# sunwj/SunVolumeRender

Measured on AMD Instinct MI355X. Metric: Msamples/sec (paths x spp) at 1024^2 on 512^3 volume, higher is better.
Workload: dtype f32; 1 GPU; c3: 512^3 u16 CT-like volume, 1024x1024 image, 3 area lights, env map on, trace depth 1, 256 spp per step; math=bit-exact contract, parallelism=single GPU

## Files before the change

sunvolumerender_amd/csrc/svr_api.hip:

```cpp
#include "../../include/svr_abi.h"
#include "svr_kernels.hpp"
#include "svr_denoise.hpp"
#include "svr_noise.hpp"
#include "svr_project.hpp"
#include "svr_slice.hpp"
#include "svr_hits.hpp"
#include "svr_device.hpp"

#include <hip/hip_runtime.h>
#include <algorithm>
#include <cmath>
#include <cstdarg>
#include <cstdio>
#include <cstdlib>
#include <cstring>
#include <dlfcn.h>
#include <mutex>
#include <string>
#include <unordered_map>
#include <vector>

static_assert(sizeof(svr_vec3) == 12, "glm::vec3 layout");
static_assert(sizeof(svr_bbox) == 36, "cudaBBox layout");
static_assert(sizeof(svr_volume) == 112 && offsetof(svr_volume, tex) == 40 && offsetof(svr_volume, densityScale) == 48 &&
// ... 91 lines not shown
        uint32_t first = 0, count = 0, depth = 0;
        int set = -1;
    } ahead[2];
    uint64_t content_version = 0;
    int opt_frame_ahead = 1;
#ifndef SVR_GROUP
#define SVR_GROUP 32
#endif
    static constexpr int NSETS = 4, GROUP = SVR_GROUP;
    static constexpr int AHEAD_MAX = 64;
    static constexpr uint64_t CHAIN_MIN_PATHS = 12u << 20;
    struct SlotSet {
        float* lbuf = nullptr;
        hipStream_t stream = nullptr;
        hipEvent_t traced = nullptr, resolved = nullptr;
        bool used = false;
        float4* planes[svr::WF_QUEUE_PLANES] = {};
        uint32_t* wf_counts = nullptr;
    } sets[NSETS];
    size_t queue_capacity = 0;
    size_t slot_floats = 0;
    uint32_t slots_per_set = 0;
    int next_set = 0;
    int opt_pipeline = 1, opt_refill = 16, opt_empty_skip = 1, opt_ray_skip = 1, opt_debug_stop = 0, opt_frames_log2 = -1, opt_unit = 0, opt_rc_lanes = 3, opt_bound_cull = 1, opt_park_end = 32, opt_fold = 1, opt_queue = 1, opt_fast_math = 0, opt_fine_mask = 0, opt_row_order = 0, opt_group_frames = 64, opt_local_majorant = 0, opt_light_cull = 1, opt_lm_tune = 0, opt_lm_sub = 1, opt_park_cheap = 16, opt_pinhole_fast = 1, opt_pool = 1, opt_trips = 1, opt_nan_guard = 0, opt_macro_shift_min = 0, opt_split = 0, opt_env_nee = 0, opt_fast_bound = 1;
    uint32_t* d_mask = nullptr;
    uint32_t* d_fine_mask = nullptr;
    size_t fine_mask_words = 0;
    uint8_t* d_bnd8 = nullptr;
    uint8_t* d_sub8 = nullptr;
    bool sub8_valid = false;
    bool bnd8_valid = false;
    uint8_t* d_mask_tmp = nullptr;
    uint32_t* d_pick = nullptr;
    bool mask_valid = false;
    uint64_t mask_vol = 0, mask_tf = 0, mask_tf_version = 0;
    uint32_t mask_ds_bits = 0, mask_sigma_bits = 0;
    bool mask_cull_useful = false, mask_has_empty = true;
    uint32_t mask_words = 0;
    int opt_denoise_preview = 0;
    svr_denoise_params dn = DN_DEFAULT;
    float4* d_guides = nullptr;
    size_t guides_px = 0;
    bool guides_valid = false;
    svr::DevScene guides_key{};
    uint64_t guides_vol = 0, guides_tf = 0, guides_tf_version = 0;
    float guides_h = 0.f;
    int guides_skip = -1;
// ... 519 lines not shown
        if (!st.wf_counts) HIP_TRY(hipMalloc((void**)&st.wf_counts, 64 * sizeof(uint32_t)));
    }
    if (need >= ((size_t)1 << 31)) return fail(-3, "frame too large for the wavefront queues");
    for (auto& st : g.sets)
        for (auto& p : st.planes) HIP_TRY(hipMalloc((void**)&p, need * sizeof(float4)));
    g.queue_capacity = need;
    return 0;
}

struct TileList {
    const uint32_t* list = nullptr;
    uint32_t count = 0;
    const uint8_t* active = nullptr;
};

struct LaunchPlan {
    svr::DevScene s;
    svr::LaunchCfg cfg;
    void* img = nullptr;
    const svr_render_params* rp = nullptr;
    const TileList* tiles = nullptr;
    bool fold_batch = false;
    bool use_queue = false;
    bool local_majorant = false;
    bool frame_ahead = false;
};

constexpr uint32_t FOLD_MIN = 8;

int plan_launch(LaunchPlan& p, void* img, const svr_render_params* rp, uint32_t nframes, const TileList* adaptive)
{
    svr::DevScene& s = p.s;
    svr::LaunchCfg& cfg = p.cfg;
    p.img = img;
    p.rp = rp;
    p.tiles = adaptive != nullptr && adaptive->list != nullptr ? adaptive : nullptr;
    if (build_scene(g.vol, g.tf, g.cam, s)) return g.err_code;
    if (add_lights_env(s)) return g.err_code;
    if ((size_t)3 * s.imageW * s.imageH >= ((size_t)1 << 32)) return fail(-3, "image too large");
    if (rp->frameNo == 0 && partial_frame(s.imageW, s.imageH))
        HIP_TRY(hipMemsetAsync(rp->hdrBuffer, 0, sizeof(float) * 3 * (size_t)s.imageW * s.imageH, g.stream));
    cfg.kernel = g.opt_kernel == svr::KERNEL_AUTO ? svr::KERNEL_TILE : g.opt_kernel;
    if (g.opt_env_nee && cfg.kernel == svr::KERNEL_TILE && s.env != nullptr && s.env_cdf != nullptr && s.env_on_escape && rp->traceDepth >= 2 && !g.opt_debug_stop)
        cfg.kernel = svr::KERNEL_ENV_NEE;
    if ((cfg.kernel == svr::KERNEL_TILE || cfg.kernel == svr::KERNEL_WAVEFRONT || cfg.kernel == svr::KERNEL_ENV_NEE) && ensure_mask(s, g.vol, g.tf)) return g.err_code;
    if (cfg.kernel == svr::KERNEL_WAVEFRONT) {
// ... 6 lines not shown
    cfg.frames_log2 = g.opt_frames_log2;
    cfg.unit_override = g.opt_unit;
    cfg.lm_straight = g.opt_local_majorant == 2;
    cfg.pool_primary = false;
    p.fold_batch = cfg.kernel == svr::KERNEL_TILE && g.opt_fold && !g.opt_debug_stop && cfg.frames_log2 < 0;
    p.use_queue = p.fold_batch && g.opt_queue == 2;
    if (p.fold_batch && g.opt_queue == 1 && g.opt_empty_skip) {
        svr::DevWork wq;
        fill_work(wq, s.imageW, s.imageH);
        const uint64_t waves = (uint64_t)(cfg.num_cus * cfg.blocks_per_cu) / 4u * svr::TILE_WAVES;
        p.use_queue = rp->traceDepth >= 2 || s.bound_cull || (uint64_t)wq.n_items >= svr::QUEUE_AUTO_TASKS_PER_WAVE * waves;
    }
    p.local_majorant = g.opt_local_majorant && cfg.kernel == svr::KERNEL_TILE && s.empty_mask != nullptr && s.ray_skip && !g.opt_debug_stop;
    if (p.local_majorant && !g.opt_lm_tune && rp->traceDepth > 1) s.lm_tune = 2u | (32u << 8) | (48u << 16) | (s.lm_tune & 0xff000000u);
    if (p.local_majorant) p.use_queue = false;
    cfg.pool_primary = p.use_queue && (g.opt_pool == 2 || (g.opt_pool == 1 && s.bound_cull && !s.has_empty));
    if (p.use_queue || (p.local_majorant && p.fold_batch)) {
        bool available = true;
        if (ensure_record_queues((uint32_t)(cfg.num_cus * cfg.blocks_per_cu) * 4u / 16u, g.opt_queue == 1 && !p.local_majorant, available)) return g.err_code;
        p.use_queue = p.use_queue && available;
    }
    p.frame_ahead = nframes == 1 && g.opt_frame_ahead && g.opt_pipeline && !g.opt_count && !g.opt_debug_stop && cfg.kernel == svr::KERNEL_TILE &&
                    adaptive == nullptr;
    const uint32_t tail_frames = nframes % (uint32_t)(p.fold_batch ? g.opt_group_frames : Context::GROUP);
    if ((!p.fold_batch || p.frame_ahead || (tail_frames != 0 && tail_frames < FOLD_MIN)) &&
        ensure_slots(s.imageW, s.imageH, nframes < (uint32_t)Context::GROUP ? nframes : (uint32_t)Context::GROUP)) return g.err_code;
    return 0;
}

svr::DevWork launch_work(const LaunchPlan& p, uint32_t first, uint32_t n, bool want_img)
{
    svr::DevWork w;
    fill_work(w, p.s.imageW, p.s.imageH);
    w.hdr = (float*)p.rp->hdrBuffer;
    w.img = want_img ? (uint8_t*)p.img : nullptr;
    w.traceDepth = p.rp->traceDepth;
    w.frame0 = first;
    w.nframes = n;
    if (p.tiles) {
        w.tile_list = p.tiles->list;
        w.tile_count = p.tiles->count;
        w.tile_active = p.tiles->active;
        w.row_order = 0;
    }
    return w;
}

// ... 104 lines not shown
        svr::DevWork w = launch_work(p, n, 1, want_img);
        w.slot_stride = (uint32_t)g.slot_floats;
        w.lbuf = set.lbuf + (size_t)(n - a.first) * g.slot_floats;
        HIP_TRY(hipStreamWaitEvent(g.stream, set.traced, 0));
        HIP_TRY(svr::launch_resolve(s, w, g.stream));
        HIP_TRY(hipEventRecord(set.resolved, g.stream));
        const uint32_t next_first = a.first + a.count;
        const uint32_t next_count = 2u * a.count < batch_max ? 2u * a.count : batch_max;
        if (next_count > 1u && !in_stock(g.ahead[0], next_first) && !in_stock(g.ahead[1], next_first))
            return trace_group(p, next_set(), next_first, next_count, 0, false, ahead_queue && next_count >= 16u);
        return 0;
    }
    uint32_t batch = 1;
    while (batch < batch_max && 2u * batch <= n + 1u) batch *= 2u;
    if (batch_max > 1 && ensure_slots(s.imageW, s.imageH, batch_max)) return g.err_code;
    if (trace_group(p, next_set(), n, batch, 1, want_img, ahead_queue && batch >= 16u)) return g.err_code;
    if (batch_max > 1) {
        const uint32_t next_count = 2u * batch < batch_max ? 2u * batch : batch_max;
        return trace_group(p, next_set(), n + batch, next_count, 0, false, ahead_queue && next_count >= 16u);
    }
    return 0;
}

int render_frames_traced(void* img, const svr_render_params* rp, uint32_t nframes, bool tonemap, const TileList* adaptive)
{
    if (ensure_init()) return g.err_code;
    if (!rp) return fail(-4, "render_pathtracer: renderParams is null");
    if (!g.have_vol || !g.have_tf || !g.have_cam)
        return fail(-4, "render_pathtracer before setup_volume/setup_transferfunction/setup_camera");
    if (!rp->hdrBuffer) return fail(-4, "render_pathtracer: renderParams.hdrBuffer is null (call SetupHDRBuffer)");
    if (nframes == 0) return 0;
    LaunchPlan p;
    if (plan_launch(p, img, rp, nframes, adaptive)) return g.err_code;
    const bool want_img = tonemap && !g.opt_skip_tonemap;
    if (p.frame_ahead) return render_ahead(p, want_img);
    const uint32_t group = p.fold_batch ? (uint32_t)g.opt_group_frames : (uint32_t)Context::GROUP;
    for (uint32_t g0 = 0; g0 < nframes; g0 += group) {
        const uint32_t n = nframes - g0 < group ? nframes - g0 : group;
        const bool img_now = want_img && g0 + n >= nframes;
        if (p.fold_batch && n >= FOLD_MIN) {
            if (trace_fold(p, rp->frameNo + g0, n, img_now)) return g.err_code;
        } else if (trace_group(p, next_set(), rp->frameNo + g0, n, n, img_now)) return g.err_code;
    }
    return 0;
}


int check_denoise_params(const svr_denoise_params& p)
{
    if (p.passes < 1 || p.passes > 10) return fail(-6, "svr_denoise_params.passes must be 1..10 (got %d)", p.passes);
    const float v[6] = {p.sigma_depth, p.sigma_normal, p.sigma_albedo, p.sigma_opacity, p.sigma_color, p.step};
    for (float x : v)
        if (!std::isfinite(x) || x < 0.f) return fail(-6, "svr_denoise_params: sigmas and step must be finite and >= 0");
    return 0;
}

float guide_step(const svr::DevScene& s, const svr_denoise_params& p)
{
    if (p.step > 0.f) return p.step;
    double e = 1e30;
    const double n[3] = {s.fnx, s.fny, s.fnz};
// ... 1371 lines not shown
    case SVR_OPT_KERNEL:
        if (value < 0 || value > 4) return fail(-6, "SVR_OPT_KERNEL: bad value %d", value);
        g.opt_kernel = value; return 0;
    case SVR_OPT_COUNT: g.opt_count = value ? 1 : 0; return 0;
    case SVR_OPT_TIMING: g.opt_timing = value ? 1 : 0; return 0;
    case SVR_OPT_SKIP_TONEMAP: g.opt_skip_tonemap = value ? 1 : 0; return 0;
    case SVR_OPT_DENOISE_PREVIEW:
        if (value < 0) return fail(-6, "SVR_OPT_DENOISE_PREVIEW: bad value %d (0 = off, N > 0 = frames)", value);
        g.opt_denoise_preview = value; return 0;
    case SVR_OPT_NOISE_ESTIMATE:
        if (value != 0 && value != 1) return fail(-6, "SVR_OPT_NOISE_ESTIMATE: bad value %d (0 off, 1 on)", value);
        g.opt_noise_estimate = value; return 0;
    case SVR_OPT_BLOCKS_PER_CU:
        if (value < 0 || value > 8) return fail(-6, "SVR_OPT_BLOCKS_PER_CU: bad value %d", value);
        g.opt_blocks_per_cu = value; return 0;
    case SVR_OPT_PIPELINE: g.opt_pipeline = value ? 1 : 0; return 0;
    case SVR_OPT_EMPTY_SKIP: g.opt_empty_skip = value ? 1 : 0; return 0;
    case SVR_OPT_RAY_SKIP: g.opt_ray_skip = value ? 1 : 0; return 0;
    case SVR_OPT_BOUND_CULL:
        if (value < 0 || value > 2) return fail(-6, "SVR_OPT_BOUND_CULL: bad value %d (0 off, 1 auto, 2 always)", value);
        g.opt_bound_cull = value; return 0;
    case SVR_OPT_FOLD: g.opt_fold = value ? 1 : 0; return 0;
    case SVR_OPT_GROUP_FRAMES:
        if (value != 8 && value != 16 && value != 32 && value != 64) return fail(-6, "SVR_OPT_GROUP_FRAMES: bad value %d (8, 16, 32, 64)", value);
        g.opt_group_frames = value; return 0;
    case SVR_OPT_ROW_ORDER: g.opt_row_order = value ? 1 : 0; return 0;
    case SVR_OPT_FINE_MASK:
        if (value < 0 || value > 2) return fail(-6, "SVR_OPT_FINE_MASK: bad value %d (0 off, 1 auto, 2 always)", value);
        g.opt_fine_mask = value; return 0;
    case SVR_OPT_FAST_MATH: g.opt_fast_math = value ? 1 : 0; g.ahead[0].valid = g.ahead[1].valid = false; return 0;
    case SVR_OPT_LIGHT_CULL: g.opt_light_cull = value ? 1 : 0; return 0;
    case SVR_OPT_LM_SUBCELLS:
        if (value < 0 || value > 2) return fail(-6, "SVR_OPT_LM_SUBCELLS: bad value %d (0 off, 1 auto, 2 always)", value);
        g.opt_lm_sub = value; g.ahead[0].valid = g.ahead[1].valid = false; return 0;
    case SVR_OPT_LM_TUNE: {
        const int steps = value & 0xff, refill = (value >> 8) & 0xff, ended = (value >> 16) & 0xff, tasks = (value >> 24) & 0x7f;
        if (value != 0 && (steps < 1 || steps > 64 || refill < 1 || refill > 64 || ended < 1 || ended > 64 || tasks > 23 || value < 0)) return fail(-6, "SVR_OPT_LM_TUNE: bad value 0x%x (cells per turn | idle lanes << 8 | ended walks << 16, each 1..64, | tasks per batch of the depth-1 pool << 24, 0 = default .. 23)", value);
        g.opt_lm_tune = value; return 0;
    }
    case SVR_OPT_LOCAL_MAJORANT:
        if (value < 0 || value > 2) return fail(-6, "SVR_OPT_LOCAL_MAJORANT: bad value %d (0 off, 1 on, 2 on with straight-line paths only)", value);
        g.opt_local_majorant = value; g.ahead[0].valid = g.ahead[1].valid = false; return 0;
    case SVR_OPT_QUEUE:
        if (value < 0 || value > 2) return fail(-6, "SVR_OPT_QUEUE: bad value %d (0 off, 1 auto, 2 always)", value);
        g.opt_queue = value; g.queue_alloc_failed = false; return 0;
    case SVR_OPT_PINHOLE_FAST: g.opt_pinhole_fast = value ? 1 : 0; return 0;
    case SVR_OPT_POOL:
// ... 239 lines not shown
```

sunvolumerender_amd/csrc/svr_primary.hpp:

```cpp
#pragma once
#include "svr_walk.hpp"
#include "svr_lanes.hpp"

namespace svr {

#ifndef SVR_SHADOW_REMARCH
#define SVR_SHADOW_REMARCH true
#endif
#ifndef SVR_PRIMARY_REMARCH
#define SVR_PRIMARY_REMARCH false
#endif

template <int LAYOUT, bool COUNT, bool SKIP, bool SHARE = false, typename LDS>
SVR_DEV bool trace_primary(const DevScene& s, const LDS& L_, uint32_t x, uint32_t y, uint32_t hashed, bool group_march, uint32_t P2,
                           GroupMapShared* gslot, Cnt& c, Rng& rng, v3& L, v3& pt, v3& wo, float& val, const DevScene* scp = nullptr, uint32_t fg = 0u,
                           uint32_t* march_did = nullptr)
{
    const DevScene& sc = scp ? *scp : s;
    uint32_t offset = y * sc.imageW + x;
    rng_init(rng, hashed + offset);
    if (COUNT) c.paths++;
    L = V3(0.f, 0.f, 0.f);
    const v3 T = V3(1.f, 1.f, 1.f);
    v3 orig, dir;
    camera_ray(sc, x, y, rng, orig, dir);
    float ls_t;
    int ls_id = nearest_light(sc, orig, dir, ls_t);
    float tMin = (float)1e-6, tMax = SVR_FLT_MAX;
    val = 0.f;
    float t;
    if (SKIP && group_march) {
        float t_occ;
        GroupMap map;
        map.g = gslot + ((threadIdx.x & 63u) & ((1u << P2) - 1u) & (GROUP_MAPS_PER_WAVE - 1u));
        int r;
        bool shared = false;
        if constexpr (SHARE && SVR_MARCH_BLOCK > 1) shared = P2 == 0u && sc.cam_pinhole != 0u;
        if (shared)
            r = walk_setup_shared<COUNT, SKIP>(s, sc, L_, x, y, fg, orig, dir, false, tMin, tMax, t_occ, gslot, map, march_did);
        else
            r = walk_setup_group<COUNT, SKIP>(s, L_, P2, orig, dir, false, tMin, tMax, t_occ, map);
        t = r <= 0 ? -SVR_FLT_MAX
                   : walk_run<LAYOUT, COUNT, SKIP, false, true>(s, L_, orig, dir, rng, tMin, tMax, t_occ, val, false, c, &map, P2);
    } else
        t = walk<LAYOUT, COUNT, SKIP, SVR_PRIMARY_REMARCH>(s, L_, orig, dir, rng, tMin, tMax, val, false, c);
    if (ls_id >= 0) {
        float tt = t < 0.f ? SVR_FLT_MAX : t;
        if (ls_t < tt) {
            const DevLight& l = sc.lights[ls_id];
            float cosTerm = dot(V3(l.normal[0], l.normal[1], l.normal[2]), -dir);
            L = L + (T * V3(l.radiance[0], l.radiance[1], l.radiance[2])) * (cosTerm <= 0.f ? 0.f : 1.f);
            return false;
        }
    }
    if (t < 0.f) {
        if (sc.env_on_escape) L = L + T * env_radiance(sc, dir);
        return false;
    }
    wo = -dir;
    pt = orig + dir * t;
    return true;
}
// ... 34 lines not shown
```

sunvolumerender_amd/csrc/svr_selftest.hip:

```cpp
#include "svr_kernels.hpp"
#include "svr_device.hpp"
#include "svr_walk.hpp"
#include "svr_chain.hpp"

namespace svr {

__global__ __launch_bounds__(256) void k_math_selftest(int fn, const float* __restrict__ in, uint32_t stride, float* __restrict__ out, uint32_t n)
{
    const uint32_t i = blockIdx.x * 256u + threadIdx.x;
    if (i >= n) return;
    const float* a = in + (size_t)i * stride;
    const float x = a[0], y = stride > 1 ? a[1] : 0.f, z = stride > 2 ? a[2] : 0.f;
    float r = 0.f, sn, cs;
    switch (fn) {
    case 0: r = schlick_fresnel(x, y, z); break;
    case 1: r = logf_(x); break;
    case 2: r = expf_(x); break;
    case 3: sincosf_(x, &sn, &cs); r = sn; break;
    case 4: sincosf_(x, &sn, &cs); r = cs; break;
    case 5: r = acosf_(x); break;
    case 6: r = atan2f_(x, y); break;
    case 7: r = powf_(x, y); break;
    case 8: {
        Rng g;
// ... 54 lines not shown
    }
    return hipGetLastError();
}

__global__ __launch_bounds__(256) void k_group_march_selftest(const DevScene s, uint32_t frame0, unsigned long long* __restrict__ out)
{
    __shared__ LdsTileCull lds;
    __shared__ GroupMapShared gmaps[4][GROUP_MAPS_PER_WAVE];
    lds_tile_load(lds, s, true);
    const uint32_t lane = threadIdx.x & 63u, wave = threadIdx.x >> 6;
    GroupMapShared* gslot = &gmaps[wave][0];
    march_kept_reset(gslot);
    unsigned long long n_bad = 0, n_pts = 0, n_hit = 0, n_valid = 0, n_did[5] = {0, 0, 0, 0, 0};
    const uint32_t hashed = wang_hash(frame0 + lane);
    for (uint32_t y = blockIdx.x * 4u + wave; y < s.imageH; y += gridDim.x * 4u) {
        for (uint32_t x = 0; x < s.imageW; ++x) {
            Rng rng;
            rng_init(rng, hashed + (y * s.imageW + x));
            v3 orig, dir;
            camera_ray(s, x, y, rng, orig, dir);
            float tMin, tMax, t_occ;
            GroupMap map;
            uint32_t did = MARCH_NONE;
            const int r = walk_setup_shared<true, true>(s, s, lds, x, y, 0u, orig, dir, false, tMin, tMax, t_occ, gslot, map, &did);
            n_did[did]++;
            const float bmax = fmax_(__builtin_fabsf(dir.x * s.mc_scale[0]), fmax_(__builtin_fabsf(dir.y * s.mc_scale[1]), __builtin_fabsf(dir.z * s.mc_scale[2])));
            if (r >= 0) { n_hit++; if (map.valid) n_valid++; }
            const float dtc = 0.125f / bmax;
            float clear_until = t_occ;
            for (uint32_t i = 0; i < 65536u && r >= 0 && bmax > 0.f; ++i) {
                const float t = fma_((float)i, dtc, tMin);
                if (t > tMax) break;
                if (t >= clear_until && map.valid) {
                    const float nx = group_map_next(map, 0u, t);
                    if (nx > t) clear_until = nx;
                    continue;
                }
                if (t >= clear_until) continue;
                const Cell c = cell_of(s, orig + dir * t);
                const uint32_t ux = (uint32_t)(c.cx + 1), uy = (uint32_t)(c.cy + 1), uz = (uint32_t)(c.cz + 1);
                if (!((ux <= (uint32_t)s.nx) & (uy <= (uint32_t)s.ny) & (uz <= (uint32_t)s.nz))) continue;
                n_pts++;
                if (!cell_is_empty<false>(lds, s, c)) n_bad++;
            }
        }
    }
    const unsigned long long tot[4] = {wave_sum(n_bad), wave_sum(n_pts), wave_sum(n_hit), wave_sum(n_valid)};
// ... 33 lines not shown
```

sunvolumerender_amd/csrc/svr_tile_tasks.hpp:

```cpp
#pragma once
#include "svr_kernel_common.hpp"

namespace svr {

#ifndef SVR_TILE_LIST
#define SVR_TILE_LIST 0
#endif

struct TaskShape {
    uint32_t tiles_x, tiles_y, fgroups, row_tasks, c_row, tw2, th2, P2, fl2, wv, n_tasks;
#if SVR_TILE_LIST
    const uint32_t* list;
#endif
};

__host__ __device__ inline uint32_t launch_tasks(const DevWork& w, uint32_t tw2, uint32_t th2, uint32_t fgroups)
{
#if SVR_TILE_LIST
    if (w.tile_list != nullptr) return (w.tile_count << ((4u - tw2) + (4u - th2))) * fgroups;
#endif
    return (((w.x1 - w.x0) + (1u << tw2) - 1u) >> tw2) * ((w.n_rows + (1u << th2) - 1u) >> th2) * fgroups;
}

SVR_DEV TaskShape task_shape(const DevWork& w)
// ... 51 lines not shown
struct TaskLanes { uint32_t px, r, slot; bool live; };
SVR_DEV TaskLanes task_lanes(const TaskShape& ts, const DevWork& w, uint32_t k, uint32_t lane)
{
    uint32_t tx, ty, fg;
    task_decode(ts, k, tx, ty, fg);
    const uint32_t pl = lane & ((1u << ts.P2) - 1u);
    TaskLanes t;
    t.slot = (fg << ts.fl2) + (lane >> ts.P2);
    t.px = (tx << ts.tw2) + (pl & ((1u << ts.tw2) - 1u));
    t.r = (ty << ts.th2) + (pl >> ts.tw2);
    t.live = t.px < ts.wv && t.r < w.n_rows && t.slot < w.nframes;
    return t;
}

struct TaskGrid { uint32_t n_tasks, blocks; };
inline hipError_t task_launch_setup(const DevWork& w, const LaunchCfg& cfg, uint32_t waves_per_block, bool fold, int frames_log2, hipStream_t st,
                                    DevWork& w2, TaskGrid& g)
{
    uint32_t fl2 = 0;
    while (fl2 < 6u && (2u << fl2) <= w.nframes) ++fl2;
    if (frames_log2 >= 0 && (uint32_t)frames_log2 < fl2) fl2 = (uint32_t)frames_log2;
    if (fold) {
        fl2 = 0;
        while ((1u << fl2) < w.nframes) ++fl2;
    }
    const uint32_t P2 = 6u - fl2, tw2 = (P2 + 1u) >> 1, th2 = P2 >> 1;
    const uint32_t fgroups = (w.nframes + (1u << fl2) - 1u) >> fl2;
    g.n_tasks = launch_tasks(w, tw2, th2, fgroups);
    const uint32_t max_blocks = (uint32_t)(cfg.num_cus * cfg.blocks_per_cu) * 4u / waves_per_block;
    g.blocks = (g.n_tasks + waves_per_block - 1u) / waves_per_block;
    if (g.blocks > max_blocks) g.blocks = max_blocks;
    if (g.blocks == 0) g.blocks = 1;
    w2 = w;
    w2.unit = 1u;
    w2.frames_log2 = fl2;
    return hipMemsetAsync(w.ticket, 0, sizeof(uint32_t) * TICKET_SHARDS * TICKET_STRIDE, st);
}

#ifndef SVR_FOLD_LOAD_AHEAD
#define SVR_FOLD_LOAD_AHEAD 1
#endif
constexpr uint32_t FOLD_CHUNK = 8;
template <bool AHEAD = true>
SVR_DEV void fold_pending(const DevScene& s, const DevWork& w, const float* rows, uint32_t row, const uint32_t* tasks, uint32_t npend)
{
    const TaskShape ts = task_shape(w);
    const uint32_t lane = threadIdx.x & 63u;
// ... 24 lines not shown
            uint32_t f = 0;
            if constexpr (AHEAD && SVR_FOLD_LOAD_AHEAD) {
                for (; f + FOLD_CHUNK <= nfr; f += FOLD_CHUNK) {
                    float Lv[FOLD_CHUNK];
#pragma unroll
                    for (uint32_t j = 0; j < FOLD_CHUNK; ++j) Lv[j] = rp[(f + j) << ts.P2];
#pragma unroll
                    for (uint32_t j = 0; j < FOLD_CHUNK; ++j) {
                        const float n1 = (float)(w.frame0 + f + j) + 1.f;
                        acc = acc + (Lv[j] - acc) / n1;
                    }
                }
            }
            for (; f < nfr; ++f) {
                const float Lf = rp[f << ts.P2];
                const float n1 = (float)(w.frame0 + f) + 1.f;
                acc = acc + (Lf - acc) / n1;
            }
        }
        *h = acc;
    }
}

SVR_DEV void direct_put(const DevScene& s, const DevWork& w, const uint32_t* tasks, uint32_t id, v3 L)
{
    const TaskShape ts = task_shape(w);
    uint32_t tx, ty, fg;
    task_decode(ts, tasks[id >> 6], tx, ty, fg);
    const uint32_t ln = id & 63u, pl = ln & ((1u << ts.P2) - 1u), fs = ln >> ts.P2;
    const uint32_t px = (tx << ts.tw2) + (pl & ((1u << ts.tw2) - 1u));
    const uint32_t r = (ty << ts.th2) + (pl >> ts.tw2);
    const uint32_t x = w.x0 + px, y = owned_row_to_y(w, r), slot = (fg << ts.fl2) + fs;
    float* o = w.lbuf + (size_t)slot * w.slot_stride + 3 * ((size_t)y * s.imageW + x);
    o[0] = L.x; o[1] = L.y; o[2] = L.z;
}

}
```

sunvolumerender_amd/csrc/svr_trace_tile.hip:

```cpp
#include "svr_walk.hpp"
#include "svr_lanes.hpp"
#include "svr_tile_tasks.hpp"
#include "svr_primary.hpp"

namespace svr {

#ifdef SVR_TEST_HOOKS
#define SVR_DEBUG_STOPS 1
#else
#define SVR_DEBUG_STOPS 0
#endif

#ifndef SVR_SHADOW_REMARCH
#define SVR_SHADOW_REMARCH true
#endif
#ifndef SVR_PRIMARY_REMARCH
#define SVR_PRIMARY_REMARCH false
#endif

template <int LAYOUT, bool COUNT, bool SKIP, bool DEPTH1, typename LDS>
SVR_DEV v3 trace_path_tile(const DevScene& s, const LDS& L_, uint32_t x, uint32_t y, uint32_t traceDepth_,
                           uint32_t hashed, uint32_t debug_stop, bool group_march, uint32_t P2, GroupMapShared* gslot, Cnt& c)
{
    const uint32_t traceDepth = DEPTH1 ? 1u : traceDepth_;
// ... 143 lines not shown
    const uint32_t lane = threadIdx.x & 63u;
    const uint32_t wave = threadIdx.x >> 6;
#ifndef SVR_COLD_SCENE
#define SVR_COLD_SCENE 1
#endif
    auto cold_scene = [&]() -> const DevScene* {
        if constexpr (QUEUE && (DEPTH1 || (POOL && SVR_COLD_DEEP_POOL) || SVR_COLD_DEEP_ALL) && SVR_COLD_SCENE) {
            auto p = __builtin_amdgcn_kernarg_segment_ptr();
            asm volatile("" : "+s"(p));
            return (const DevScene*)p;
        } else return nullptr;
    };
    const TaskShape ts = task_shape(w);
    const uint32_t fl2 = ts.fl2, P2 = ts.P2, tw2 = ts.tw2, th2 = ts.th2, wv = ts.wv, fgroups = ts.fgroups;
    const uint32_t n_tasks = ts.n_tasks;
    Cnt c = {0, 0, 0, 0, 0, 0, 0, 0, 0, 0};
    constexpr bool SHARE = Drain::WIDE && !SVR_TILE_LIST && SVR_MARCH_BLOCK > 1;
    if constexpr (SHARE) march_kept_reset(&gmaps[wave][0]);

    const uint32_t unit = w.unit;
    const uint32_t n_units = (n_tasks + unit - 1u) / unit;
    const uint32_t shard0 = blockIdx.x % TICKET_SHARDS;
    const bool fold = w.fold != 0u;
    uint32_t npend = 0, qC = 0, qA = 0, qB = 0;
    LaneQueue Q;
    Q.cap = DRAIN_CAP;
    Q.q = QUEUE ? w.queue + (size_t)(blockIdx.x * TILE_WAVES + wave) * (REC_WORDS * DRAIN_CAP) : nullptr;
    float* const gpend = QUEUE ? w.pend + (size_t)(blockIdx.x * TILE_WAVES + wave) * (DRAIN_TASKS * 3u * 64u) : nullptr;
    auto flush = [&]() {
        if constexpr (QUEUE) {
            __builtin_amdgcn_fence(__ATOMIC_RELEASE, "workgroup");
            __builtin_amdgcn_fence(__ATOMIC_ACQUIRE, "workgroup");
            if constexpr (POOL && !DEPTH1) {
                static_assert(REC_C1_WORDS <= REC_A_WORDS, "P records lie in front of the B stack");
                uint32_t nH = 0u;
                drain_queue<LAYOUT, COUNT, SKIP, true, LDS, true, true, DIRECT, LDSL>(s, lds, Q, qC, 0u, 0u, 1u, gpend, 64u, c, w.counters + CNT_N, true, &nH, &w, &pend.task[wave][0], cold_scene(), lts);
                __builtin_amdgcn_fence(__ATOMIC_RELEASE, "workgroup");
                __builtin_amdgcn_fence(__ATOMIC_ACQUIRE, "workgroup");
                qC = 0u; qA = 0u; qB = nH;
            } else if constexpr (POOL) {
                uint32_t nH = 0u;
                drain_queue<LAYOUT, COUNT, SKIP, DEPTH1, LDS, true, false, DIRECT, LDSL>(s, lds, Q, qC, 0u, 0u, 1u, gpend, 64u, c, w.counters + CNT_N, true, &nH, &w, &pend.task[wave][0], cold_scene(), lts);
                __builtin_amdgcn_fence(__ATOMIC_RELEASE, "workgroup");
                __builtin_amdgcn_fence(__ATOMIC_ACQUIRE, "workgroup");
                qC = 0u;
                for (uint32_t i0 = 0u; i0 < nH; i0 += 64u) {
// ... 14 lines not shown
                        shade_event<LAYOUT, COUNT, LDSL>(s, vs, val, rng, ne, c, cold_scene(), lts);
                        have = ne.have;
                        if (!have) {
                            if constexpr (DIRECT) direct_put(s, w, &pend.task[wave][0], id, V3(0.f, 0.f, 0.f));
                            else {
                                float* o = gpend + (id >> 6) * (3u * 64u) + (id & 63u);
                                o[0] = 0.f; o[64] = 0.f; o[128] = 0.f;
                            }
                        }
                    }
                    queue_push_c1(Q, qC, have, vs.pt, ne, rng, id);
                }
                __builtin_amdgcn_fence(__ATOMIC_RELEASE, "workgroup");
                __builtin_amdgcn_fence(__ATOMIC_ACQUIRE, "workgroup");
            }
            drain_queue<LAYOUT, COUNT, SKIP, DEPTH1, LDS, false, false, DIRECT, LDSL, FIRST>(s, lds, Q, qC, qA, qB, w.traceDepth, gpend, 64u, c, w.counters + CNT_N, false, nullptr, &w, &pend.task[wave][0], cold_scene(), lts);
            qC = qA = qB = 0;
            __builtin_amdgcn_fence(__ATOMIC_RELEASE, "workgroup");
            __builtin_amdgcn_fence(__ATOMIC_ACQUIRE, "workgroup");
#if SVR_PROF
            unsigned long long* c_prof = w.counters + CNT_N;
#endif
            PROF_BEGIN(pfo, PH_FOLD);
            if constexpr (!DIRECT) fold_pending<DEPTH1>(s, w, gpend, 64u, &pend.task[wave][0], npend);
            PROF_END(pfo, min(64u, npend * (3u << ts.P2)));
        } else {
            __builtin_amdgcn_fence(__ATOMIC_RELEASE, "wavefront");
            __builtin_amdgcn_fence(__ATOMIC_ACQUIRE, "wavefront");
            fold_pending<false>(s, w, &pend.L[wave][0][0], PEND_ROW, &pend.task[wave][0], npend);
        }
        npend = 0;
    };

#if SVR_PROF
    unsigned long long* c_prof = w.counters + CNT_N;
#endif
    PROF_BEGIN(ploop, PH_LOOP);
    for (uint32_t si = 0; si < TICKET_SHARDS; ++si) {
        const uint32_t shard = (shard0 + si) % TICKET_SHARDS;
        uint32_t* ticket = w.ticket + shard * TICKET_STRIDE;
        for (;;) {
            const uint32_t rows_s = (w.row_order && ts.tiles_y > shard) ? (ts.tiles_y - shard + TICKET_SHARDS - 1u) / TICKET_SHARDS : 0u;
            const uint32_t limit = w.row_order ? rows_s * ts.row_tasks : n_units;
            if (si != 0u && (w.row_order ? __atomic_load_n(ticket, __ATOMIC_RELAXED) : __atomic_load_n(ticket, __ATOMIC_RELAXED) * TICKET_SHARDS + shard) >= limit) break;
            PROF_BEGIN(ptk, PH_TICKET);
            uint32_t u = 0;
            if (lane == 0) u = atomicAdd(ticket, 1u);
// ... 49 lines not shown
                    }
                    if (lane == 0) pend.task[wave][npend] = k;
                    if (++npend == DRAIN_TASKS || qC + 64u > DRAIN_CAP) flush();
                    continue;
                } else if constexpr (QUEUE) {
                    Rng rng = {0u, 0u, 0u, 0u, 0u, 0u};
                    v3 L = V3(0.f, 0.f, 0.f);
                    bool hit = false;
                    float val = 0.f;
                    Shade vs;
                    vs.pt = L; vs.wo = L; vs.gradient = L; vs.color[0] = vs.color[1] = vs.color[2] = vs.color[3] = 0.f; vs.Pbrdf = 0.f; vs.st = 0;
                    Nee ne;
                    ne.wi = L; ne.B = L; ne.pdf = 1.f; ne.light = 0u; ne.have = false;
#if SVR_PROF
                    unsigned long long* c_prof = w.counters + CNT_N;
#endif
                    PROF_BEGIN(pa, PH_PRIMARY);
#if SVR_PROF
                    const uint32_t prof_i0 = c.iters - c.iskip;
#endif
                    uint32_t march_did = MARCH_NONE;
                    if (live) {
                        uint32_t x = w.x0 + px, y = owned_row_to_y(w, r);
                        hit = trace_primary<LAYOUT, COUNT, SKIP, SHARE>(s, lds, x, y, wang_hash(w.frame0 + slot), group_march, P2, &gmaps[wave][0], c, rng, L, vs.pt, vs.wo, val, cold_scene(), fg,
                                                                              SVR_PROF ? &march_did : nullptr);
                    }
#if SVR_PROF
                    if (lane == 0 && march_did != MARCH_NONE) atomicAdd(&c_prof[PROF_MARCH + march_did - 1u], 1ull);
#endif
                    PROF_END(pa, (uint32_t)__popcll(__ballot(live)));
#if SVR_PROF
                    if (COUNT && DEPTH1) {
                        const uint32_t d = (c.iters - c.iskip) - prof_i0;
                        uint32_t m = d;
                        for (int o = 32; o > 0; o >>= 1) m = max(m, (uint32_t)__shfl_xor((int)m, o));
                        const unsigned long long sum = wave_sum(d);
                        if (lane == 0) { atomicAdd(&c_prof[2 * PH_N], (unsigned long long)m * 64ull); atomicAdd(&c_prof[2 * PH_N + 1], sum); }
                    }
#endif
                    const bool shade_here = DEPTH1 || !s.bound_cull;
                    {
                        const uint64_t mh = __ballot(hit);
                        if (shade_here && mh != 0ull) {
                            PROF_BEGIN(psh, PH_SHADE);
                            if (hit) {
                                const DevScene* scp = cold_scene();
                                shade_event<LAYOUT, COUNT, LDSL>(s, vs, val, rng, ne, c, scp, lts);
// ... 82 lines not shown
                            o[0] = L.x; o[1] = L.y; o[2] = L.z;
                        }
                    }
                    if (fold) {
                        float* pl_row = &pend.L[wave][npend * 3u][lane];
                        pl_row[0] = L.x; pl_row[PEND_ROW] = L.y; pl_row[2u * PEND_ROW] = L.z;
                        if (lane == 0) pend.task[wave][npend] = k;
                        if (++npend == PEND_TASKS) flush();
                    }
                }
            }
        }
    }
    if (npend) flush();
    PROF_END(ploop, 64u);
    if (COUNT) cnt_flush(w, c);
}

template <int LAYOUT, bool COUNT>
static hipError_t launch_tile_t(const DevScene& s, const DevWork& w, const LaunchCfg& cfg, hipStream_t st)
{
    uint32_t wv = w.x1 - w.x0;
    if (wv == 0 || w.n_rows == 0) return hipSuccess;
    if (w.fold && w.nframes > 64u) return hipErrorInvalidValue;
    DevWork w2;
    TaskGrid g;
    hipError_t e = task_launch_setup(w, cfg, SVR_TILE_THREADS / 64, w.fold != 0u, cfg.frames_log2, st, w2, g);
    if (e != hipSuccess) return e;
    const uint32_t blocks = g.blocks;
    const bool skip = s.empty_mask != nullptr, d1 = w.traceDepth == 1u;
    const bool queue = LAYOUT != LAYOUT_LINEAR && w.queue != nullptr && w.pend != nullptr && blocks <= w.queue_blocks && w.traceDepth < 32768u &&
                       (w.fold || !COUNT);
    if (SVR_MARCH_BLOCK > 1 && !SVR_TILE_LIST && queue && skip && d1 && !cfg.pool_primary && w2.frames_log2 == 6u && w.nframes <= 64u && s.cam_pinhole && s.ray_skip)
        w2.unit = SVR_MARCH_BLOCK;
    if (cfg.unit_override > 0) w2.unit = (uint32_t)cfg.unit_override;
#define SVR_LAUNCH_TILE(SK, D1, QU) hipLaunchKernelGGL((k_trace_tile<LAYOUT, COUNT, SK, D1, QU>), dim3(blocks), dim3(SVR_TILE_THREADS), 0, st, s, w2)
    if constexpr (LAYOUT != LAYOUT_LINEAR && !COUNT) {
        if (queue && !w.fold) {
#define SVR_LAUNCH_DIRECT(SK, D1, PO) hipLaunchKernelGGL((k_trace_tile<LAYOUT, false, SK, D1, true, PO, true>), dim3(blocks), dim3(SVR_TILE_THREADS), 0, st, s, w2)
            if (skip && cfg.pool_primary) { if (d1) SVR_LAUNCH_DIRECT(true, true, true); else SVR_LAUNCH_DIRECT(true, false, true); }
            else if (skip && d1) SVR_LAUNCH_DIRECT(true, true, false);
            else if (skip) SVR_LAUNCH_DIRECT(true, false, false);
            else if (d1) SVR_LAUNCH_DIRECT(false, true, false);
            else SVR_LAUNCH_DIRECT(false, false, false);
#undef SVR_LAUNCH_DIRECT
            return hipGetLastError();
        }
    }
    if constexpr (LAYOUT != LAYOUT_LINEAR) {
        if (queue && skip && cfg.pool_primary) {
            if (d1) hipLaunchKernelGGL((k_trace_tile<LAYOUT, COUNT, true, true, true, true>), dim3(blocks), dim3(SVR_TILE_THREADS), 0, st, s, w2);
            else hipLaunchKernelGGL((k_trace_tile<LAYOUT, COUNT, true, false, true, true>), dim3(blocks), dim3(SVR_TILE_THREADS), 0, st, s, w2);
            return hipGetLastError();
        }
        if (queue) {
            if (skip && d1) SVR_LAUNCH_TILE(true, true, true);
            else if (skip) SVR_LAUNCH_TILE(true, false, true);
            else if (d1) SVR_LAUNCH_TILE(false, true, true);
// ... 21 lines not shown
```

sunvolumerender_amd/csrc/svr_walk.hpp:

```cpp
#pragma once
#include "svr_kernel_common.hpp"
#include <type_traits>

namespace svr {

struct LdsTile {
    float alpha[SVR_TF_MAX + SVR_TF_PAD];
    uint32_t dist[DIST_WORDS_MAX];
    uint32_t mask[MASK_WORDS_MAX];
    uint32_t emask[MASK_WORDS_MAX];
};
struct LdsTileNoMask {
    float alpha[SVR_TF_MAX + SVR_TF_PAD];
    uint32_t dist[1];
    uint32_t mask[1];
    uint32_t emask[1];
};
struct LdsTileCull : LdsTile {
    uint32_t cls[DIST_WORDS_MAX];
    float thr[BOUND_CLASSES];
};
struct LdsBound8 {
    uint8_t bnd[BOUND8_BYTES];
};
// ... 349 lines not shown
    map.lo = lo; map.dt = dt; map.inv_dt = bmax * (1.f / 0.7f);
    map.valid = complete && ok;
    __builtin_amdgcn_fence(__ATOMIC_RELEASE, "wavefront");
    __builtin_amdgcn_fence(__ATOMIC_ACQUIRE, "wavefront");
    return result;
}

#ifndef SVR_MARCH_BLOCK
#define SVR_MARCH_BLOCK 2
#endif
static_assert(SVR_MARCH_BLOCK == 1 || SVR_MARCH_BLOCK == 2, "march blocks: 1 (every pixel marches) or 2 (2 x 1 pixels)");
template <bool MAX>
SVR_DEV float wave_minmax(float v)
{
    for (int off = 32; off > 0; off >>= 1) { const float o = __shfl_xor(v, off, 64); v = MAX ? fmax_(v, o) : fmin_(v, o); }
    return v;
}

struct MarchKept {
    enum { TAG = 0, RESULT, LO, HI, DT, INV_DT, OX, OY, OZ, DX, DY, DZ, COMPLETE, WORDS };
};
static_assert(MarchKept::WORDS * 4u <= 2u * sizeof(GroupMapShared) && GROUP_MAPS_PER_WAVE >= 3u, "the kept march fits into slots 1 and 2");
constexpr uint32_t MARCH_TAG_NONE = 0xffffffffu;
SVR_DEV uint32_t march_tag(uint32_t x, uint32_t y, uint32_t fg) { return (((y << 15) ^ (x >> 1)) + fg * 0x9e3779b1u) & 0x7fffffffu; }
SVR_DEV void march_kept_reset(GroupMapShared* gslot)
{
    reinterpret_cast<uint32_t*>(gslot + 1)[MarchKept::TAG] = MARCH_TAG_NONE;
    __builtin_amdgcn_fence(__ATOMIC_RELEASE, "wavefront");
    __builtin_amdgcn_fence(__ATOMIC_ACQUIRE, "wavefront");
}

enum MarchDid : uint32_t { MARCH_NONE = 0, MARCH_SHARED, MARCH_REUSED, MARCH_REFUSED, MARCH_ALONE };

template <bool COUNT, bool SKIP, typename LDS>
SVR_DEV int walk_setup_shared(const DevScene& s, const DevScene& sc, const LDS& L, uint32_t x, uint32_t y, uint32_t fg, v3 orig, v3 dir, bool rng_live,
                              float& tMin, float& tMax, float& t_occ, GroupMapShared* gslot, GroupMap& map, uint32_t* did = nullptr)
{
    map.g = gslot;
    map.valid = false; map.lo = 0.f; map.dt = 1.f; map.inv_dt = 1.f;
    float tNear, tFar;
    const bool hit = volume_intersect(s, orig, dir, tNear, tFar);
    tMin = tNear < 0.f ? (float)1e-6 : tNear;
    tMax = tFar;
    t_occ = tMin;
    if (did) *did = MARCH_NONE;
    if (!(SKIP && s.ray_skip)) return hit ? 1 : -1;
    if (__ballot(hit) == 0ull) return -1;
    const float INF = u2f(SVR_INF_BITS);
    uint32_t* kw = reinterpret_cast<uint32_t*>(gslot + 1);
    const uint32_t tag = march_tag(x, y, fg);
    float g = INF;
    bool ok = false, complete = false, have = false;
    if (kw[MarchKept::TAG] == tag) {
        const v3 oc = V3(u2f(kw[MarchKept::OX]), u2f(kw[MarchKept::OY]), u2f(kw[MarchKept::OZ]));
        const v3 dc = V3(u2f(kw[MarchKept::DX]), u2f(kw[MarchKept::DY]), u2f(kw[MarchKept::DZ]));
        const float lo = u2f(kw[MarchKept::LO]), hi = u2f(kw[MarchKept::HI]);
        ok = group_admit(s, orig, dir, oc, dc, hi) && tMin >= lo && tMax <= hi;
        if (__ballot(hit && !ok) == 0ull) {
            have = true;
            g = u2f(kw[MarchKept::RESULT]);
            complete = kw[MarchKept::COMPLETE] != 0u;
            map.lo = lo; map.dt = u2f(kw[MarchKept::DT]); map.inv_dt = u2f(kw[MarchKept::INV_DT]);
            if (did) *did = MARCH_REUSED;
        } else if (did) *did = MARCH_REFUSED;
    }
    if (!have) {
        const bool fresh = kw[MarchKept::TAG] != tag;
        float lo = wave_minmax<false>(hit ? tMin : INF), hi = wave_minmax<true>(hit ? tMax : -INF);
        v3 oc = V3(u2f((uint32_t)__builtin_amdgcn_readfirstlane((int)f2u(orig.x))), u2f((uint32_t)__builtin_amdgcn_readfirstlane((int)f2u(orig.y))),
                   u2f((uint32_t)__builtin_amdgcn_readfirstlane((int)f2u(orig.z))));
        v3 dc = V3(0.f, 0.f, 0.f);
        bool shared = false;
        if (fresh) {
// ... 186 lines not shown
```

Before: 10960 Msamples/s.

## Fold multiple 64-frame groups per launch and reuse kept march across groups

Raises the default fold group size from 64 to 256 frames. When the depth-1, pinhole, queued tile path applies, one launch now covers several 64-frame groups, with the work unit scaled so one wave handles consecutive frame groups of a pixel pair. Drops the frame-group term from the kept-march tag so a pixel pair's empty-space march can be reused across those groups. Adds a grouped fold routine that accumulates consecutive pending groups into the HDR buffer in order. The aim is to cut launch count and repeated marching and HDR read-modify-write, at the cost of more complex fold scheduling and a possible change in load balance.

```diff
diff --git a/sunvolumerender_amd/csrc/svr_api.hip b/sunvolumerender_amd/csrc/svr_api.hip
--- a/sunvolumerender_amd/csrc/svr_api.hip
+++ b/sunvolumerender_amd/csrc/svr_api.hip
@@ -137,7 +137,7 @@
     size_t slot_floats = 0;
     uint32_t slots_per_set = 0;
     int next_set = 0;
-    int opt_pipeline = 1, opt_refill = 16, opt_empty_skip = 1, opt_ray_skip = 1, opt_debug_stop = 0, opt_frames_log2 = -1, opt_unit = 0, opt_rc_lanes = 3, opt_bound_cull = 1, opt_park_end = 32, opt_fold = 1, opt_queue = 1, opt_fast_math = 0, opt_fine_mask = 0, opt_row_order = 0, opt_group_frames = 64, opt_local_majorant = 0, opt_light_cull = 1, opt_lm_tune = 0, opt_lm_sub = 1, opt_park_cheap = 16, opt_pinhole_fast = 1, opt_pool = 1, opt_trips = 1, opt_nan_guard = 0, opt_macro_shift_min = 0, opt_split = 0, opt_env_nee = 0, opt_fast_bound = 1;
+    int opt_pipeline = 1, opt_refill = 16, opt_empty_skip = 1, opt_ray_skip = 1, opt_debug_stop = 0, opt_frames_log2 = -1, opt_unit = 0, opt_rc_lanes = 3, opt_bound_cull = 1, opt_park_end = 32, opt_fold = 1, opt_queue = 1, opt_fast_math = 0, opt_fine_mask = 0, opt_row_order = 0, opt_group_frames = 256, opt_local_majorant = 0, opt_light_cull = 1, opt_lm_tune = 0, opt_lm_sub = 1, opt_park_cheap = 16, opt_pinhole_fast = 1, opt_pool = 1, opt_trips = 1, opt_nan_guard = 0, opt_macro_shift_min = 0, opt_split = 0, opt_env_nee = 0, opt_fast_bound = 1;
     uint32_t* d_mask = nullptr;
     uint32_t* d_fine_mask = nullptr;
     size_t fine_mask_words = 0;
@@ -703,6 +703,7 @@
     const TileList* tiles = nullptr;
     bool fold_batch = false;
     bool use_queue = false;
+    bool fold_groups = false;
     bool local_majorant = false;
     bool frame_ahead = false;
 };
@@ -755,7 +756,9 @@
     }
     p.frame_ahead = nframes == 1 && g.opt_frame_ahead && g.opt_pipeline && !g.opt_count && !g.opt_debug_stop && cfg.kernel == svr::KERNEL_TILE &&
                     adaptive == nullptr;
-    const uint32_t tail_frames = nframes % (uint32_t)(p.fold_batch ? g.opt_group_frames : Context::GROUP);
+    p.fold_groups = p.fold_batch && p.use_queue && !p.local_majorant && !cfg.pool_primary && p.tiles == nullptr && rp->traceDepth == 1 &&
+                    s.empty_mask != nullptr && s.layout != svr::LAYOUT_LINEAR && s.cam_pinhole && s.ray_skip && !g.opt_row_order && !p.frame_ahead;
+    const uint32_t tail_frames = nframes % (uint32_t)(p.fold_batch ? (g.opt_group_frames < 64 ? g.opt_group_frames : 64) : Context::GROUP);
     if ((!p.fold_batch || p.frame_ahead || (tail_frames != 0 && tail_frames < FOLD_MIN)) &&
         ensure_slots(s.imageW, s.imageH, nframes < (uint32_t)Context::GROUP ? nframes : (uint32_t)Context::GROUP)) return g.err_code;
     return 0;
@@ -906,6 +909,18 @@
     return 0;
 }
 
+uint32_t fold_group_frames(const LaunchPlan& p, uint32_t left)
+{
+    const uint32_t group = (uint32_t)g.opt_group_frames;
+    if (group <= 64u || left < 128u || !p.fold_groups) {
+        const uint32_t cap = group < 64u ? group : 64u;
+        return left < cap ? left : cap;
+    }
+    const uint32_t n = (left < group ? left : group) & ~63u;
+    if (g.opt_unit > 0 && (uint32_t)g.opt_unit % (n >> 6) != 0u) return 64u;
+    return n;
+}
+
 int render_frames_traced(void* img, const svr_render_params* rp, uint32_t nframes, bool tonemap, const TileList* adaptive)
 {
     if (ensure_init()) return g.err_code;
@@ -918,9 +933,8 @@
     if (plan_launch(p, img, rp, nframes, adaptive)) return g.err_code;
     const bool want_img = tonemap && !g.opt_skip_tonemap;
     if (p.frame_ahead) return render_ahead(p, want_img);
-    const uint32_t group = p.fold_batch ? (uint32_t)g.opt_group_frames : (uint32_t)Context::GROUP;
-    for (uint32_t g0 = 0; g0 < nframes; g0 += group) {
-        const uint32_t n = nframes - g0 < group ? nframes - g0 : group;
+    for (uint32_t g0 = 0, n = 0; g0 < nframes; g0 += n) {
+        n = p.fold_batch ? fold_group_frames(p, nframes - g0) : (nframes - g0 < (uint32_t)Context::GROUP ? nframes - g0 : (uint32_t)Context::GROUP);
         const bool img_now = want_img && g0 + n >= nframes;
         if (p.fold_batch && n >= FOLD_MIN) {
             if (trace_fold(p, rp->frameNo + g0, n, img_now)) return g.err_code;
@@ -2338,7 +2352,8 @@
         g.opt_bound_cull = value; return 0;
     case SVR_OPT_FOLD: g.opt_fold = value ? 1 : 0; return 0;
     case SVR_OPT_GROUP_FRAMES:
-        if (value != 8 && value != 16 && value != 32 && value != 64) return fail(-6, "SVR_OPT_GROUP_FRAMES: bad value %d (8, 16, 32, 64)", value);
+        if (value != 8 && value != 16 && value != 32 && value != 64 && value != 128 && value != 256)
+            return fail(-6, "SVR_OPT_GROUP_FRAMES: bad value %d (8, 16, 32, 64, 128, 256)", value);
         g.opt_group_frames = value; return 0;
     case SVR_OPT_ROW_ORDER: g.opt_row_order = value ? 1 : 0; return 0;
     case SVR_OPT_FINE_MASK:
diff --git a/sunvolumerender_amd/csrc/svr_primary.hpp b/sunvolumerender_amd/csrc/svr_primary.hpp
--- a/sunvolumerender_amd/csrc/svr_primary.hpp
+++ b/sunvolumerender_amd/csrc/svr_primary.hpp
@@ -13,7 +13,7 @@
 
 template <int LAYOUT, bool COUNT, bool SKIP, bool SHARE = false, typename LDS>
 SVR_DEV bool trace_primary(const DevScene& s, const LDS& L_, uint32_t x, uint32_t y, uint32_t hashed, bool group_march, uint32_t P2,
-                           GroupMapShared* gslot, Cnt& c, Rng& rng, v3& L, v3& pt, v3& wo, float& val, const DevScene* scp = nullptr, uint32_t fg = 0u,
+                           GroupMapShared* gslot, Cnt& c, Rng& rng, v3& L, v3& pt, v3& wo, float& val, const DevScene* scp = nullptr,
                            uint32_t* march_did = nullptr)
 {
     const DevScene& sc = scp ? *scp : s;
@@ -37,7 +37,7 @@
         bool shared = false;
         if constexpr (SHARE && SVR_MARCH_BLOCK > 1) shared = P2 == 0u && sc.cam_pinhole != 0u;
         if (shared)
-            r = walk_setup_shared<COUNT, SKIP>(s, sc, L_, x, y, fg, orig, dir, false, tMin, tMax, t_occ, gslot, map, march_did);
+            r = walk_setup_shared<COUNT, SKIP>(s, sc, L_, x, y, orig, dir, false, tMin, tMax, t_occ, gslot, map, march_did);
         else
             r = walk_setup_group<COUNT, SKIP>(s, L_, P2, orig, dir, false, tMin, tMax, t_occ, map);
         t = r <= 0 ? -SVR_FLT_MAX
diff --git a/sunvolumerender_amd/csrc/svr_selftest.hip b/sunvolumerender_amd/csrc/svr_selftest.hip
--- a/sunvolumerender_amd/csrc/svr_selftest.hip
+++ b/sunvolumerender_amd/csrc/svr_selftest.hip
@@ -100,7 +100,7 @@
             float tMin, tMax, t_occ;
             GroupMap map;
             uint32_t did = MARCH_NONE;
-            const int r = walk_setup_shared<true, true>(s, s, lds, x, y, 0u, orig, dir, false, tMin, tMax, t_occ, gslot, map, &did);
+            const int r = walk_setup_shared<true, true>(s, s, lds, x, y, orig, dir, false, tMin, tMax, t_occ, gslot, map, &did);
             n_did[did]++;
             const float bmax = fmax_(__builtin_fabsf(dir.x * s.mc_scale[0]), fmax_(__builtin_fabsf(dir.y * s.mc_scale[1]), __builtin_fabsf(dir.z * s.mc_scale[2])));
             if (r >= 0) { n_hit++; if (map.valid) n_valid++; }
diff --git a/sunvolumerender_amd/csrc/svr_tile_tasks.hpp b/sunvolumerender_amd/csrc/svr_tile_tasks.hpp
--- a/sunvolumerender_amd/csrc/svr_tile_tasks.hpp
+++ b/sunvolumerender_amd/csrc/svr_tile_tasks.hpp
@@ -97,7 +97,7 @@
     if (frames_log2 >= 0 && (uint32_t)frames_log2 < fl2) fl2 = (uint32_t)frames_log2;
     if (fold) {
         fl2 = 0;
-        while ((1u << fl2) < w.nframes) ++fl2;
+        while (fl2 < 6u && (1u << fl2) < w.nframes) ++fl2;
     }
     const uint32_t P2 = 6u - fl2, tw2 = (P2 + 1u) >> 1, th2 = P2 >> 1;
     const uint32_t fgroups = (w.nframes + (1u << fl2) - 1u) >> fl2;
@@ -168,6 +168,62 @@
     }
 }
 
+SVR_DEV void fold_pending_groups(const DevScene& s, const DevWork& w, const float* rows, const uint32_t* tasks, uint32_t npend)
+{
+    const TaskShape ts = task_shape(w);
+    const uint32_t lane = threadIdx.x & 63u;
+    const bool mine = lane < npend;
+    const uint32_t k_l = mine ? tasks[lane] : 0u, k_p = (mine && lane != 0u) ? tasks[lane - 1u] : 0u;
+    uint32_t tx_l, ty_l, fg_l;
+    task_decode(ts, k_l, tx_l, ty_l, fg_l);
+    const bool head = mine && (lane == 0u || fg_l == 0u || k_p + 1u != k_l);
+    const uint64_t heads = __ballot(head);
+    const uint32_t nheads = (uint32_t)__popcll(heads);
+    const uint32_t rank = (uint32_t)__popcll(heads & ((1ull << lane) - 1ull));
+    const uint32_t dest = head ? rank : nheads + (lane - rank);
+    const uint32_t q_of = (uint32_t)__builtin_amdgcn_ds_permute((int)(dest << 2), (int)lane);
+    const uint32_t items = nheads * 3u;
+    for (uint32_t i0 = 0u; i0 < items; i0 += 64u) {
+        const uint32_t i = i0 + lane;
+        const uint32_t j = (i * 0xAAABu) >> 17;
+        const uint32_t ch = i - 3u * j;
+        const uint32_t q = (uint32_t)__shfl((int)q_of, (int)(j & 63u), 64);
+        if (i >= items) continue;
+        uint32_t tx, ty, fg;
+        task_decode(ts, tasks[q], tx, ty, fg);
+        if (tx >= ts.wv || ty >= w.n_rows) continue;
+        const uint64_t above = q < 63u ? heads >> (q + 1u) : 0ull;
+        const uint32_t len = above ? (uint32_t)__builtin_ctzll(above) + 1u : npend - q;
+        const uint32_t x = w.x0 + tx, y = owned_row_to_y(w, ty);
+        float* h = w.hdr + 3 * ((size_t)y * s.imageW + x) + ch;
+        float acc = (w.frame0 == 0u && fg == 0u) ? 0.f : *h;
+        for (uint32_t gi = 0u; gi < len; ++gi) {
+            const float* rp = rows + (size_t)((q + gi) * 3u + ch) * 64u;
+            const uint32_t n0 = w.frame0 + ((fg + gi) << 6);
+            if (w.nan_guard) {
+                for (uint32_t f = 0; f < 64u; ++f) {
+                    float Lf = rp[f];
+                    Lf = (f2u(Lf) & 0x7f800000u) == 0x7f800000u ? acc : Lf;
+                    const float n1 = (float)(n0 + f) + 1.f;
+                    acc = acc + (Lf - acc) / n1;
+                }
+            } else {
+                for (uint32_t f = 0; f < 64u; f += FOLD_CHUNK) {
+                    float Lv[FOLD_CHUNK];
+#pragma unroll
+                    for (uint32_t jj = 0; jj < FOLD_CHUNK; ++jj) Lv[jj] = rp[f + jj];
+#pragma unroll
+                    for (uint32_t jj = 0; jj < FOLD_CHUNK; ++jj) {
+                        const float n1 = (float)(n0 + f + jj) + 1.f;
+                        acc = acc + (Lv[jj] - acc) / n1;
+                    }
+                }
+            }
+        }
+        *h = acc;
+    }
+}
+
 SVR_DEV void direct_put(const DevScene& s, const DevWork& w, const uint32_t* tasks, uint32_t id, v3 L)
 {
     const TaskShape ts = task_shape(w);
diff --git a/sunvolumerender_amd/csrc/svr_trace_tile.hip b/sunvolumerender_amd/csrc/svr_trace_tile.hip
--- a/sunvolumerender_amd/csrc/svr_trace_tile.hip
+++ b/sunvolumerender_amd/csrc/svr_trace_tile.hip
@@ -189,6 +189,7 @@
     const uint32_t n_units = (n_tasks + unit - 1u) / unit;
     const uint32_t shard0 = blockIdx.x % TICKET_SHARDS;
     const bool fold = w.fold != 0u;
+    constexpr bool GROUPS = Drain::WIDE && !DIRECT && !SVR_TILE_LIST;
     uint32_t npend = 0, qC = 0, qA = 0, qB = 0;
     LaneQueue Q;
     Q.cap = DRAIN_CAP;
@@ -249,7 +250,10 @@
             unsigned long long* c_prof = w.counters + CNT_N;
 #endif
             PROF_BEGIN(pfo, PH_FOLD);
-            if constexpr (!DIRECT) fold_pending<DEPTH1>(s, w, gpend, 64u, &pend.task[wave][0], npend);
+            if constexpr (GROUPS) {
+                if (fgroups > 1u) fold_pending_groups(s, w, gpend, &pend.task[wave][0], npend);
+                else fold_pending<DEPTH1>(s, w, gpend, 64u, &pend.task[wave][0], npend);
+            } else if constexpr (!DIRECT) fold_pending<DEPTH1>(s, w, gpend, 64u, &pend.task[wave][0], npend);
             PROF_END(pfo, min(64u, npend * (3u << ts.P2)));
         } else {
             __builtin_amdgcn_fence(__ATOMIC_RELEASE, "wavefront");
@@ -345,7 +349,7 @@
                     uint32_t march_did = MARCH_NONE;
                     if (live) {
                         uint32_t x = w.x0 + px, y = owned_row_to_y(w, r);
-                        hit = trace_primary<LAYOUT, COUNT, SKIP, SHARE>(s, lds, x, y, wang_hash(w.frame0 + slot), group_march, P2, &gmaps[wave][0], c, rng, L, vs.pt, vs.wo, val, cold_scene(), fg,
+                        hit = trace_primary<LAYOUT, COUNT, SKIP, SHARE>(s, lds, x, y, wang_hash(w.frame0 + slot), group_march, P2, &gmaps[wave][0], c, rng, L, vs.pt, vs.wo, val, cold_scene(),
                                                                               SVR_PROF ? &march_did : nullptr);
                     }
 #if SVR_PROF
@@ -474,7 +478,8 @@
 {
     uint32_t wv = w.x1 - w.x0;
     if (wv == 0 || w.n_rows == 0) return hipSuccess;
-    if (w.fold && w.nframes > 64u) return hipErrorInvalidValue;
+    const bool many_groups = w.fold && w.nframes > 64u;
+    if (many_groups && ((w.nframes & 63u) != 0u || cfg.frames_log2 >= 0)) return hipErrorInvalidValue;
     DevWork w2;
     TaskGrid g;
     hipError_t e = task_launch_setup(w, cfg, SVR_TILE_THREADS / 64, w.fold != 0u, cfg.frames_log2, st, w2, g);
@@ -483,9 +488,13 @@
     const bool skip = s.empty_mask != nullptr, d1 = w.traceDepth == 1u;
     const bool queue = LAYOUT != LAYOUT_LINEAR && w.queue != nullptr && w.pend != nullptr && blocks <= w.queue_blocks && w.traceDepth < 32768u &&
                        (w.fold || !COUNT);
-    if (SVR_MARCH_BLOCK > 1 && !SVR_TILE_LIST && queue && skip && d1 && !cfg.pool_primary && w2.frames_log2 == 6u && w.nframes <= 64u && s.cam_pinhole && s.ray_skip)
-        w2.unit = SVR_MARCH_BLOCK;
+    const bool wide_form = !SVR_TILE_LIST && queue && skip && d1 && !cfg.pool_primary && w2.frames_log2 == 6u && s.cam_pinhole && s.ray_skip;
+    const uint32_t fgroups = (w.nframes + 63u) >> 6;
+    if (many_groups && !(wide_form && !w.row_order)) return hipErrorInvalidValue;
+    if (wide_form && (many_groups || (SVR_MARCH_BLOCK > 1 && w.nframes <= 64u)))
+        w2.unit = SVR_MARCH_BLOCK * (many_groups ? fgroups : 1u);
     if (cfg.unit_override > 0) w2.unit = (uint32_t)cfg.unit_override;
+    if (many_groups && w2.unit % fgroups != 0u) return hipErrorInvalidValue;
 #define SVR_LAUNCH_TILE(SK, D1, QU) hipLaunchKernelGGL((k_trace_tile<LAYOUT, COUNT, SK, D1, QU>), dim3(blocks), dim3(SVR_TILE_THREADS), 0, st, s, w2)
     if constexpr (LAYOUT != LAYOUT_LINEAR && !COUNT) {
         if (queue && !w.fold) {
diff --git a/sunvolumerender_amd/csrc/svr_walk.hpp b/sunvolumerender_amd/csrc/svr_walk.hpp
--- a/sunvolumerender_amd/csrc/svr_walk.hpp
+++ b/sunvolumerender_amd/csrc/svr_walk.hpp
@@ -395,7 +395,7 @@
 };
 static_assert(MarchKept::WORDS * 4u <= 2u * sizeof(GroupMapShared) && GROUP_MAPS_PER_WAVE >= 3u, "the kept march fits into slots 1 and 2");
 constexpr uint32_t MARCH_TAG_NONE = 0xffffffffu;
-SVR_DEV uint32_t march_tag(uint32_t x, uint32_t y, uint32_t fg) { return (((y << 15) ^ (x >> 1)) + fg * 0x9e3779b1u) & 0x7fffffffu; }
+SVR_DEV uint32_t march_tag(uint32_t x, uint32_t y) { return ((y << 15) ^ (x >> 1)) & 0x7fffffffu; }
 SVR_DEV void march_kept_reset(GroupMapShared* gslot)
 {
     reinterpret_cast<uint32_t*>(gslot + 1)[MarchKept::TAG] = MARCH_TAG_NONE;
@@ -406,7 +406,7 @@
 enum MarchDid : uint32_t { MARCH_NONE = 0, MARCH_SHARED, MARCH_REUSED, MARCH_REFUSED, MARCH_ALONE };
 
 template <bool COUNT, bool SKIP, typename LDS>
-SVR_DEV int walk_setup_shared(const DevScene& s, const DevScene& sc, const LDS& L, uint32_t x, uint32_t y, uint32_t fg, v3 orig, v3 dir, bool rng_live,
+SVR_DEV int walk_setup_shared(const DevScene& s, const DevScene& sc, const LDS& L, uint32_t x, uint32_t y, v3 orig, v3 dir, bool rng_live,
                               float& tMin, float& tMax, float& t_occ, GroupMapShared* gslot, GroupMap& map, uint32_t* did = nullptr)
 {
     map.g = gslot;
@@ -421,7 +421,7 @@
     if (__ballot(hit) == 0ull) return -1;
     const float INF = u2f(SVR_INF_BITS);
     uint32_t* kw = reinterpret_cast<uint32_t*>(gslot + 1);
-    const uint32_t tag = march_tag(x, y, fg);
+    const uint32_t tag = march_tag(x, y);
     float g = INF;
     bool ok = false, complete = false, have = false;
     if (kw[MarchKept::TAG] == tag) {
```

Result: faster. 11870 Msamples/s (median of 6 runs) (+8.3%).
